# wpats/scanner

Hardware: AMD Instinct MI355X
Metric: Msamples/s (complex samples through convert->window->FFT->dB->threshold) (higher is better)
Workload: dtype f32

## Files before the change

### scanner_amd/csrc/scn_device.h

```cpp
#pragma once
#include <hip/hip_runtime.h>
#include <stdint.h>

#include "scn_kernels.h"

typedef scn_v2f v2f;
typedef float v16f __attribute__((ext_vector_type(16)));

__device__ __forceinline__ cf operator+(cf a, cf b) { return cf{a.x + b.x, a.y + b.y}; }
__device__ __forceinline__ cf operator-(cf a, cf b) { return cf{a.x - b.x, a.y - b.y}; }
__device__ __forceinline__ cf operator*(cf a, float s) { return cf{a.x * s, a.y * s}; }
__device__ __forceinline__ cf from_v2f(v2f v) { return cf{v.x, v.y}; }
__device__ __forceinline__ v2f to_v2f(cf c) { return v2f{c.x, c.y}; }

namespace {

#define SCN_P_EXACT_FROM 1584.8932f
__device__ __forceinline__ float db_fast(float p) { return 1.50514997831990597607f * __builtin_amdgcn_logf(p); }
__device__ __forceinline__ float db_exact(float p) {
  const float m = __builtin_amdgcn_frexp_mantf(p);
  const float e = (float)__builtin_amdgcn_frexp_expf(p);
  const float KH = 1.505126953125f;
  const float KL = (float)(1.50514997831990597607 - 1.505126953125);
  return __builtin_fmaf(KL, e, __builtin_fmaf(1.50514997831990597607f, __builtin_amdgcn_logf(m), KH * e));
// ... 88 lines not shown
  v[14] = mul_w6_d(v[14], H);
  v[7] = cmul_d(v[7], S1, -C1);
  v[11] = mul_w6_d(v[11], H);
  v[15] = cmul_d(v[15], -C1, S1);
#pragma unroll
  for (int k0 = 0; k0 < 4; k0++) radix4_d(v[4 * k0], v[4 * k0 + 1], v[4 * k0 + 2], v[4 * k0 + 3]);
}

__device__ __forceinline__ __amdgpu_buffer_rsrc_t make_rsrc(const void *p, uint32_t bytes) {
  return __builtin_amdgcn_make_buffer_rsrc(const_cast<void *>(p), 0, bytes, 0x00020000);
}
constexpr int SCN_AUX_LD = 2;
constexpr int SCN_AUX_ST = 2;

__device__ __forceinline__ int wave_sum(int v) {
#pragma unroll
  for (int off = 32; off > 0; off >>= 1) v += __shfl_xor(v, off, 64);
  return v;
}

#define SCN_DPP_STEP(OP, x, ctrl, rmask) x = x OP (uint32_t)__builtin_amdgcn_update_dpp(0, (int)x, ctrl, rmask, 0xf, true)
__device__ __forceinline__ uint32_t wave_or_u32(uint32_t x) {
  SCN_DPP_STEP(|, x, 0x111, 0xf);
  SCN_DPP_STEP(|, x, 0x112, 0xf);
  SCN_DPP_STEP(|, x, 0x114, 0xf);
  SCN_DPP_STEP(|, x, 0x118, 0xf);
  SCN_DPP_STEP(|, x, 0x142, 0xa);
  SCN_DPP_STEP(|, x, 0x143, 0xc);
  return (uint32_t)__builtin_amdgcn_readlane((int)x, 63);
}
__device__ __forceinline__ uint32_t wave_add_u32(uint32_t x) {
  SCN_DPP_STEP(+, x, 0x111, 0xf);
  SCN_DPP_STEP(+, x, 0x112, 0xf);
  SCN_DPP_STEP(+, x, 0x114, 0xf);
  SCN_DPP_STEP(+, x, 0x118, 0xf);
  SCN_DPP_STEP(+, x, 0x142, 0xa);
  SCN_DPP_STEP(+, x, 0x143, 0xc);
  return (uint32_t)__builtin_amdgcn_readlane((int)x, 63);
}

template <int NB, typename VEC, typename ARGS, typename BINI>
__device__ __forceinline__ void scn_record_hits_device_counter(VEC &pw, const float (&gmax)[4], uint32_t keepmask, const ARGS &args, int *count,
                                                               uint32_t buf, uint32_t lane, BINI bin_i) {
  constexpr int GS = NB / 4;
  uint32_t wmc = 0;
#pragma unroll
  for (int g = 0; g < 4; g++) {
    if (__ballot(gmax[g] > args.p_lo)) {
#pragma unroll
      for (int o = g * GS; o < (g + 1) * GS; o++) wmc |= __ballot(pw[o] > args.p_lo) ? (1u << o) : 0u;
    }
  }
  ScnDevHit *const region = args.hits + (size_t)buf * args.hit_region;
  uint32_t hm = 0, wm2 = 0, total = 0;
  while (wmc) {
    const int o = __builtin_ctz(wmc);
    wmc &= wmc - 1u;
    const float p = pw[o];
    float d = db_fast(p);
    if (__ballot(p >= SCN_P_EXACT_FROM)) d = p >= SCN_P_EXACT_FROM ? db_exact(p) : d;
    const bool hit = ((keepmask >> o) & 1u) && d > args.threshold && p > args.p_lo;
    const unsigned long long m = __ballot(hit);
    pw[o] = d;
    hm |= hit ? (1u << o) : 0u;
    wm2 |= m ? (1u << o) : 0u;
    total += (uint32_t)__popcll(m);
  }
  if (!total) return;
  uint32_t base = 0;
  if (lane == 0) base = (uint32_t)atomicAdd(count, (int)total);
  base = (uint32_t)__builtin_amdgcn_readfirstlane((int)base);
  while (wm2) {
    const int o = __builtin_ctz(wm2);
    wm2 &= wm2 - 1u;
    const bool hit = (hm >> o) & 1u;
    const unsigned long long m = __ballot(hit);
    if (hit) {
      const uint32_t pos = base + (uint32_t)__popcll(m & ((1ull << lane) - 1ull));
      if (pos < args.hit_region) region[pos] = ScnDevHit{bin_i(o), pw[o]};
    }
    base += (uint32_t)__popcll(m);
  }
}

__device__ __forceinline__ float scn_cndmask(float a, float b, unsigned long long m) {
  float r;
  asm("v_cndmask_b32 %0, %1, %2, %3" : "=v"(r) : "v"(a), "v"(b), "s"(m));
  return r;
}
template <int NB, typename VEC>
__device__ __forceinline__ float scn_select_output(const VEC &pw, uint32_t o) {
  float t[NB / 2];
  const unsigned long long m0 = __ballot(o & 1u);
#pragma unroll
  for (int i = 0; i < NB / 2; i++) t[i] = scn_cndmask(pw[2 * i], pw[2 * i + 1], m0);
#pragma unroll
  for (int w = NB / 4, bit = 1; w >= 1; w >>= 1, bit++) {
    const unsigned long long m = __ballot((o >> bit) & 1u);
#pragma unroll
    for (int i = 0; i < w; i++) t[i] = scn_cndmask(t[2 * i], t[2 * i + 1], m);
  }
  return t[0];
}

template <int T, int NB, typename VEC, typename ARGS, typename BINI>
__device__ __forceinline__ uint32_t scn_record_hits_segment(const VEC &dbv, uint32_t hm, const ARGS &args, uint32_t buf, uint32_t t, BINI bin_i) {
  static_assert(T >= 1 && T <= 32 && (T & (T - 1)) == 0, "a segment is a power of two of lanes inside a wave");
  const uint32_t cnt = (uint32_t)__builtin_popcount(hm);
  uint32_t inc = cnt;
#pragma unroll
  for (int off = 1; off < T; off <<= 1) {
    const uint32_t v = (uint32_t)__shfl_up((int)inc, off, T);
    inc += t >= (uint32_t)off ? v : 0u;
  }
  const uint32_t total = T == 1 ? inc : (uint32_t)__shfl((int)inc, T - 1, T);
  uint32_t pos = inc - cnt;
  ScnDevHit *const region = args.hits + (size_t)buf * args.hit_region;
  while (__ballot(hm != 0u)) {
    const bool act = hm != 0u;
    const uint32_t o = act ? (uint32_t)__builtin_ctz(hm) : 0u;
    hm &= hm - 1u;
    const float d = scn_select_output<NB>(dbv, o);
    if (act && pos < args.hit_region) region[pos] = ScnDevHit{bin_i((int)o), d};
    pos += 1u;
  }
  return total;
}

template <int NB, bool IS_DB, bool PURE = false, bool HAVE_MASK = false, typename VEC, typename ARGS, typename BINI>
__device__ __forceinline__ void scn_record_hits_lanes(VEC &pw, const float (&gmax)[4], uint32_t keepmask, const ARGS &args, int *count, uint32_t buf,
                                                      uint32_t lane, BINI bin_i, uint32_t cand = 0) {
  constexpr int GS = NB / 4;
  uint32_t hm = cand;
  if constexpr (!HAVE_MASK) {
#pragma unroll
    for (int g = 0; g < 4; g++) {
      if (__ballot(gmax[g] > args.p_lo)) {
#pragma unroll
        for (int o = g * GS; o < (g + 1) * GS; o++) hm |= (IS_DB ? pw[o] > args.threshold : pw[o] > args.p_lo) ? (1u << o) : 0u;
      }
    }
  }
  hm &= keepmask;
  ScnDevHit *const region = args.hits + (size_t)buf * args.hit_region;
  if constexpr (IS_DB) {
    const uint32_t cnt = (uint32_t)__builtin_popcount(hm);
    uint32_t inc = cnt;
    SCN_DPP_STEP(+, inc, 0x111, 0xf);
    SCN_DPP_STEP(+, inc, 0x112, 0xf);
    SCN_DPP_STEP(+, inc, 0x114, 0xf);
    SCN_DPP_STEP(+, inc, 0x118, 0xf);
    SCN_DPP_STEP(+, inc, 0x142, 0xa);
    SCN_DPP_STEP(+, inc, 0x143, 0xc);
    const uint32_t total = (uint32_t)__builtin_amdgcn_readlane((int)inc, 63);
    if (!total) return;
    uint32_t base = 0;
    if (lane == 0) base = (uint32_t)atomicAdd(count, (int)total);
    uint32_t pos = (uint32_t)__builtin_amdgcn_readfirstlane((int)base) + inc - cnt;
    while (__ballot(hm != 0u)) {
      const bool act = hm != 0u;
      const uint32_t o = act ? (uint32_t)__builtin_ctz(hm) : 0u;
      hm &= hm - 1u;
      const float d = scn_select_output<NB>(pw, o);
      if (act && pos < args.hit_region) region[pos] = ScnDevHit{bin_i((int)o), d};
      pos += 1u;
    }
    return;
  }
  while (__ballot(hm != 0u)) {
    const bool act = hm != 0u;
    const uint32_t o = act ? (uint32_t)__builtin_ctz(hm) : 0u;
    hm &= hm - 1u;
    const float p = scn_select_output<NB>(pw, o);
    float d = p;
    if constexpr (!IS_DB) {
      d = db_fast(p);
      if constexpr (PURE) {
        const bool ex = p >= SCN_P_EXACT_FROM;
        if (__ballot(act && ex)) d = ex ? db_exact(p) : d;
      } else {
        const float gm = scn_select_output<4>(gmax, o / GS);
        const bool ex = gm >= SCN_P_EXACT_FROM && d == db_fast(gm);
        if (__ballot(act && ex)) d = ex ? db_exact(gm) : d;
      }
    }
    const bool hit = act && d > args.threshold && (IS_DB || p > args.p_lo);
    const unsigned long long m = __ballot(hit);
    if (m) {
      const int first = __builtin_ctzll(m);
      uint32_t base = 0;
      if (lane == (uint32_t)first) base = (uint32_t)atomicAdd(count, (int)__popcll(m));
      base = (uint32_t)__builtin_amdgcn_readlane((int)base, first);
      if (hit) {
        const uint32_t pos = base + (uint32_t)__popcll(m & ((1ull << lane) - 1ull));
        if (pos < args.hit_region) region[pos] = ScnDevHit{bin_i((int)o), d};
      }
    }
  }
}

template <int NB, typename VEC, typename SOFF>
__device__ __forceinline__ void scn_store_exact_db(const VEC &pw, const float (&gmax)[4], float pmax, __amdgpu_buffer_rsrc_t rout, uint32_t st_voff,
                                                   SOFF soff_of) {
  constexpr int GS = NB / 4;
  if (__ballot(pmax >= SCN_P_EXACT_FROM)) {
#pragma unroll
    for (int g = 0; g < 4; g++) {
      if (__ballot(gmax[g] >= SCN_P_EXACT_FROM)) {
#pragma unroll
        for (int o = g * GS; o < (g + 1) * GS; o++) {
          const float q = pw[o];
          if (__ballot(q >= SCN_P_EXACT_FROM)) {
            const float d = db_exact(q);
            __builtin_amdgcn_raw_buffer_store_b32(__builtin_bit_cast(int, d), rout, q >= SCN_P_EXACT_FROM ? st_voff : 0x80000000u, soff_of(o), SCN_AUX_ST);
          }
        }
      }
    }
  }
}

template <int KIND>
struct RawLoader;

template <>
struct RawLoader<SCN_K_FLOAT_COMPLEX> : Wire<SCN_K_FLOAT_COMPLEX> {
  template <int AUX>
  static __device__ __forceinline__ raw_t load(__amdgpu_buffer_rsrc_t r, uint32_t, uint32_t t, uint32_t idx0) {
    return __builtin_bit_cast(v2f, __builtin_amdgcn_raw_buffer_load_b64(r, t * 8u, idx0 * 8u, AUX));
  }
  template <int AUX>
  static __device__ __forceinline__ void load2(__amdgpu_buffer_rsrc_t r, uint32_t, uint32_t t, uint32_t idx0, raw_t &r0, raw_t &r1) {
    typedef float v4f_t __attribute__((ext_vector_type(4)));
    const v4f_t v = __builtin_bit_cast(v4f_t, __builtin_amdgcn_raw_buffer_load_b128(r, t * 16u, idx0 * 8u, AUX));
    r0 = v2f{v.x, v.y};
    r1 = v2f{v.z, v.w};
  }
};

template <>
struct RawLoader<SCN_K_SHORT_COMPLEX> : Wire<SCN_K_SHORT_COMPLEX> {
  template <int AUX>
  static __device__ __forceinline__ raw_t load(__amdgpu_buffer_rsrc_t r, uint32_t, uint32_t t, uint32_t idx0) {
    return __builtin_amdgcn_raw_buffer_load_b32(r, t * 4u, idx0 * 4u, AUX);
  }
  template <int AUX>
  static __device__ __forceinline__ void load2(__amdgpu_buffer_rsrc_t r, uint32_t, uint32_t t, uint32_t idx0, raw_t &r0, raw_t &r1) {
    typedef int v2i_t __attribute__((ext_vector_type(2)));
    const v2i_t v = __builtin_bit_cast(v2i_t, __builtin_amdgcn_raw_buffer_load_b64(r, t * 8u, idx0 * 4u, AUX));
    r0 = v.x;
    r1 = v.y;
  }
};

template <>
struct RawLoader<SCN_K_BYTE_COMPLEX> : Wire<SCN_K_BYTE_COMPLEX> {
  template <int AUX>
  static __device__ __forceinline__ raw_t load(__amdgpu_buffer_rsrc_t r, uint32_t, uint32_t t, uint32_t idx0) {
    int v;
    const unsigned short h = __builtin_amdgcn_raw_buffer_load_b16(r, t * 2u, idx0 * 2u, AUX);
    asm("" : "=v"(v) : "0"(h));
    return v;
  }
  template <int AUX>
  static __device__ __forceinline__ void load2(__amdgpu_buffer_rsrc_t r, uint32_t, uint32_t t, uint32_t idx0, raw_t &r0, raw_t &r1) {
    const uint32_t v = (uint32_t)__builtin_amdgcn_raw_buffer_load_b32(r, t * 4u, idx0 * 2u, AUX);
    r0 = (int)(v & 0xffffu);
    r1 = (int)(v >> 16);
  }
};

template <>
struct RawLoader<SCN_K_SHORT> : Wire<SCN_K_SHORT> {
  template <int AUX>
  static __device__ __forceinline__ raw_t load(__amdgpu_buffer_rsrc_t r, uint32_t n, uint32_t t, uint32_t idx0) {
    int re = (int)(unsigned short)__builtin_amdgcn_raw_buffer_load_b16(r, t * 2u, idx0 * 2u, AUX);
    int im = (int)(unsigned short)__builtin_amdgcn_raw_buffer_load_b16(r, t * 2u, (n + idx0) * 2u, AUX);
    return (re & 0xffff) | (im << 16);
  }
  template <int AUX>
  static __device__ __forceinline__ void load2(__amdgpu_buffer_rsrc_t r, uint32_t n, uint32_t t, uint32_t idx0, raw_t &r0, raw_t &r1) {
    const uint32_t re = (uint32_t)__builtin_amdgcn_raw_buffer_load_b32(r, t * 4u, idx0 * 2u, AUX);
    const uint32_t im = (uint32_t)__builtin_amdgcn_raw_buffer_load_b32(r, t * 4u, (n + idx0) * 2u, AUX);
    r0 = (int)((re & 0xffffu) | (im << 16));
    r1 = (int)((re >> 16) | (im & 0xffff0000u));
  }
};

template <int M>
struct Geo {
  static_assert(M == 4 || M == 8 || M == 16, "1024, 2048 or 4096 points");
  static constexpr uint32_t N = 256u * M;
  static constexpr uint32_t T = 16u * M;
  static constexpr uint32_t P1 = T + M;
  static constexpr uint32_t P2 = 256u + 16u / M;
  static constexpr uint32_t EXCH = (16u * P1 > M * P2) ? 16u * P1 : M * P2;
  static constexpr uint32_t LDS_BYTES = EXCH * 8u + T * 8u + 16u * 4u + 2u * 4u + 64u * 4u + 8u;
  static constexpr uint32_t WAVES = T / 64;
  static constexpr uint32_t WAVES_PER_SIMD = 3;
  static constexpr uint32_t WG_PER_CU = (WAVES_PER_SIMD * 4u) / WAVES;
};

template <int M>
__device__ __forceinline__ constexpr int out_reg(int o) {
  return M == 4 ? o : M == 8 ? (o & ~7) + OUT8(o & 7) : OUT16(o & 15);
}

}
```

### scanner_amd/csrc/scn_kernels.hip

```cpp
#include <hip/hip_runtime.h>
#include <hip/hip_ext.h>
#include <stdint.h>
#include <stdlib.h>

#include "scn_device.h"
#include "scn_dispatch.h"
#include "scn_kernels.h"

#ifndef SCN_TU
#define SCN_TU -1
#endif
#define SCN_IN_TU(x) (SCN_TU == -1 || SCN_TU == (x))
#define SCN_TU_COUNT 8


#define SCN_WORK_QUEUE_SETUP()                                                                         \
  const uint32_t wq_shard = blockIdx.x & 7u;                                                           \
  uint32_t *const wq_head = args.work_counter + 32u * wq_shard;        \
  const uint32_t wq_base = args.work_base[wq_shard];                                                   \
  const uint32_t wq_j0 = (gridDim.x - wq_shard + 7u) >> 3;                                             \
  uint32_t wq_zero;                                                                                    \
  asm("v_mov_b32 %0, 0" : "=v"(wq_zero));                                                              \
  auto wq_take = [&]() -> uint32_t { return atomicAdd(wq_head + wq_zero, 1u); };                       \
  auto wq_buffer = [&](uint32_t taken) -> uint32_t { return 8u * (wq_j0 + (taken - wq_base)) + wq_shard; }

template <int M, int KIND, bool DC, bool HITS, bool SPEC>
__global__ __launch_bounds__(16 * M, Geo<M>::WAVES_PER_SIMD) void scn_fft_kernel(ScnFftArgs args) {
  static_assert(HITS || SPEC, "a kernel that reports nothing");
  typedef Geo<M> G;
  constexpr int AUX_LD = SCN_AUX_LD;
  constexpr int AUX_ST = SCN_AUX_ST;
  constexpr bool DYN = scn_uses_queue(KIND, G::N);
  constexpr uint32_t N = G::N, T = G::T, P1 = G::P1, P2 = G::P2;
  typedef RawLoader<KIND> L;
  extern __shared__ __attribute__((aligned(16))) char smem_raw[];
  v2f *lds = reinterpret_cast<v2f *>(smem_raw);
  v2f *lds_tw2 = lds + G::EXCH;
  int *lds_cnt = reinterpret_cast<int *>(lds_tw2 + T);
  int *lds_hits = lds_cnt + 32;
  uint32_t *lds_next = reinterpret_cast<uint32_t *>(lds_hits + 2);

  const uint32_t t = threadIdx.x;
  const uint32_t p2 = t / M, c2 = t % M;
  const uint32_t lane = t & 63, wave = t >> 6;

  typename L::raw_t raw[16];
  if (blockIdx.x < args.n_buffers) {
    __amdgpu_buffer_rsrc_t r0 = make_rsrc(reinterpret_cast<const char *>(args.raw) + (size_t)blockIdx.x * L::kBytes * N, L::kBytes * N);
#pragma unroll
    for (int a = 0; a < 16; a++) raw[a] = L::template load<AUX_LD>(r0, N, t, T * a);
  }

  cf tw1[16];
#pragma unroll
  for (int p = 1; p < 16; p++) tw1[p] = from_v2f(args.tw1_table[(p - 1) * T + t]);
  float win[16];
#pragma unroll
  for (int a = 0; a < 16; a++) win[a] = args.window[T * a + t] * args.scale;
  lds_tw2[t] = args.twiddle[(16 * p2 * c2) & (N - 1)];
  SCN_WORK_QUEUE_SETUP();
  if (t == 0) {
    lds_hits[0] = lds_hits[1] = 0;
    lds_next[0] = DYN ? wq_buffer(wq_take()) : blockIdx.x + gridDim.x;
  }
  __syncthreads();

  v2f *w1 = lds + t;
  v2f *r1 = lds + p2 * P1 + c2;
  v2f *w2 = lds + c2 * P2 + p2;
  v2f *r3 = lds + t;
  const v2f *tw2 = lds_tw2 + c2;
  const uint32_t st_voff = t * 4u;

  auto joff_of = [](int o) -> uint32_t { return T * ((uint32_t)o / M) + 256u * ((uint32_t)o % M); };
  uint32_t keepmask = 0;
  if (HITS) {
#pragma unroll
    for (int o = 0; o < 16; o++) {
      const uint32_t j = t + joff_of(o);
      const uint32_t i = j ^ (N / 2);
      const bool keep = scn_bin_evaluated(j, i, N, args);
      keepmask |= keep ? (1u << o) : 0u;
    }
  }
  uint32_t par = 0;
  uint32_t prev = 0xffffffffu;

  uint32_t buf = blockIdx.x;
  uint32_t nxt = (uint32_t)__builtin_amdgcn_readfirstlane((int)lds_next[0]);
  while (buf < args.n_buffers) {
    const bool more = nxt < args.n_buffers;
    int dc_re = 0, dc_im = 0;
    if (DC) {
      int sr = 0, si = 0;
#pragma unroll
      for (int a = 0; a < 16; a++) {
        int re, im;
        L::ints(raw[a], re, im);
        sr += re;
        si += im;
      }
      sr = wave_sum(sr);
      si = wave_sum(si);
      if (lane == 0) {
        lds_cnt[wave] = sr;
        lds_cnt[16 + wave] = si;
      }
      __syncthreads();
      sr = si = 0;
#pragma unroll
      for (uint32_t w = 0; w < G::WAVES; w++) {
        sr += lds_cnt[w];
        si += lds_cnt[16 + w];
      }
      dc_re = (int)((uint32_t)sr / N);
      dc_im = (int)((uint32_t)si / N);
    }

    cf v[16];
#pragma unroll
    for (int a = 0; a < 16; a++) v[a] = L::conv(raw[a], dc_re, dc_im, 1.0f) * win[a];
    uint32_t taken = 0;
    if (DYN && t == 0 && more) taken = wq_take();
    const __amdgpu_buffer_rsrc_t rn =
        make_rsrc(reinterpret_cast<const char *>(args.raw) + (size_t)(more ? nxt : buf) * (L::kBytes * N), more ? L::kBytes * N : 0u);
    auto prefetch = [&](int a_lo, int a_hi) {
#pragma unroll
      for (int a = 0; a < 16; a++)
        if (a >= a_lo && a < a_hi) raw[a] = L::template load<AUX_LD>(rn, N, t, T * a);
    };
    prefetch(0, 6);

    fft16(v);
#pragma unroll
    for (int p = 0; p < 16; p++) {
      cf y = v[OUT16(p)];
      if (p) y = cmul(y, tw1[p]);
      w1[p * P1] = to_v2f(y);
    }
    __syncthreads();
    if (HITS) {
      if (t == 0 && prev != 0xffffffffu) {
        args.per_buffer_hits[prev] = (uint32_t)lds_hits[par ^ 1];
        if (args.host_hits) args.host_hits[prev] = (uint32_t)lds_hits[par ^ 1];
        lds_hits[par ^ 1] = 0;
      }
    }

#pragma unroll
    for (int b = 0; b < 16; b++) v[b] = from_v2f(r1[b * M]);
    prefetch(6, 11);
    fft16(v);
#pragma unroll
    for (int q = 1; q < 16; q++) v[OUT16(q)] = cmul(v[OUT16(q)], from_v2f(tw2[q * M]));
    __syncthreads();
    prefetch(11, 16);
#pragma unroll
    for (int q = 0; q < 16; q++) w2[q * 16] = to_v2f(v[OUT16(q)]);
    __syncthreads();

#pragma unroll
    for (int u = 0; u < 16 / M; u++)
#pragma unroll
      for (int c = 0; c < M; c++) v[u * M + c] = from_v2f(r3[c * P2 + T * u]);
    if constexpr (M == 16) fft16(v);
    if constexpr (M == 8) {
      fft8(v);
      fft8(v + 8);
    }
    if constexpr (M == 4) {
#pragma unroll
      for (int u = 0; u < 4; u++) radix4(v[4 * u], v[4 * u + 1], v[4 * u + 2], v[4 * u + 3]);
    }

    v16f pw;
    float gmax[4] = {0.0f, 0.0f, 0.0f, 0.0f};
    __amdgpu_buffer_rsrc_t rout = make_rsrc(args.power_db + (size_t)buf * N, (SPEC && args.power_db) ? 4u * N : 0u);
#pragma unroll
    for (int o = 0; o < 16; o++) {
      const float q = power_of(v[out_reg<M>(o)]);
      pw[o] = q;
      gmax[o >> 2] = fmaxf(gmax[o >> 2], q);
      if constexpr (SPEC) __builtin_amdgcn_raw_buffer_store_b32(__builtin_bit_cast(int, db_fast(q)), rout, st_voff, 4u * joff_of(o), AUX_ST);
    }
    const float pmax = fmaxf(fmaxf(gmax[0], gmax[1]), fmaxf(gmax[2], gmax[3]));
    if constexpr (SPEC) scn_store_exact_db<16>(pw, gmax, pmax, rout, st_voff, [&](int o) -> uint32_t { return 4u * joff_of(o); });
    if (t == 0) lds_next[0] = !more ? 0xffffffffu : DYN ? wq_buffer(taken) : nxt + gridDim.x;
    __syncthreads();
    const uint32_t after = (uint32_t)__builtin_amdgcn_readfirstlane((int)lds_next[0]);
    if (HITS) {
      if (__ballot(pmax > args.p_lo))
        scn_record_hits_lanes<16, false, true>(pw, gmax, keepmask, args, &lds_hits[par], buf, lane, [&](int o) -> uint32_t { return (t + joff_of(o)) ^ (N / 2); });
      prev = buf;
      par ^= 1;
    }
    buf = nxt;
    nxt = after;
  }
  if (HITS) {
    __syncthreads();
    if (t == 0 && prev != 0xffffffffu) {
      args.per_buffer_hits[prev] = (uint32_t)lds_hits[par ^ 1];
      if (args.host_hits) args.host_hits[prev] = (uint32_t)lds_hits[par ^ 1];
    }
  }
}

namespace {
template <int T, bool SPEC, bool HITS, typename POWER, typename JOFF, typename STORE>
__device__ __forceinline__ void scn_small_db_store_record(POWER power_at, JOFF joff_of, STORE store, const ScnFftArgs &args, uint32_t buf, bool valid,
                                                          uint32_t keepmask, uint32_t t, uint32_t n) {
  v16f pw, dbv;
  float gmax[4] = {0.0f, 0.0f, 0.0f, 0.0f};
#pragma unroll
  for (int o = 0; o < 16; o++) {
    const float q = power_at(o);
    pw[o] = q;
    gmax[o >> 2] = fmaxf(gmax[o >> 2], q);
    if constexpr (SPEC) {
      const float d = db_fast(q);
      dbv[o] = d;
      store(o, d, true);
    }
  }
  const float pmax = fmaxf(fmaxf(gmax[0], gmax[1]), fmaxf(gmax[2], gmax[3]));
  const bool any_cand = HITS && __ballot(valid && pmax > args.p_lo) != 0ull;
  if (SPEC || any_cand) {
    if constexpr (!SPEC) {
#pragma unroll
      for (int o = 0; o < 16; o++) dbv[o] = db_fast(pw[o]);
    }
    if (__ballot(pmax >= SCN_P_EXACT_FROM)) {
#pragma unroll
      for (int g = 0; g < 4; g++) {
        if (__ballot(gmax[g] >= SCN_P_EXACT_FROM)) {
#pragma unroll
          for (int o = 4 * g; o < 4 * g + 4; o++) {
            const float q = pw[o];
            if (__ballot(q >= SCN_P_EXACT_FROM)) {
              const float d = db_exact(q);
              dbv[o] = q >= SCN_P_EXACT_FROM ? d : dbv[o];
              if constexpr (SPEC) store(o, d, q >= SCN_P_EXACT_FROM);
            }
          }
        }
      }
    }
  }
  if constexpr (HITS) {
    uint32_t total = 0;
    if (any_cand) {
      uint32_t hm = 0;
#pragma unroll
      for (int o = 0; o < 16; o++) hm |= (dbv[o] > args.threshold) ? (1u << o) : 0u;
      hm &= valid ? keepmask : 0u;
      total = scn_record_hits_segment<T, 16>(dbv, hm, args, buf, t, [&](int o) -> uint32_t { return (t + joff_of(o)) ^ (n / 2); });
    }
    if (t == 0 && valid) {
      args.per_buffer_hits[buf] = total;
      if (args.host_hits) args.host_hits[buf] = total;
    }
  }
}

template <int M>
struct GeoSmall {
  static constexpr uint32_t N = 256u * M, T = 16u * M, SLOTS = 256u / T;
  static constexpr uint32_t P1 = T + M, P2 = 256u + 16u / M;
  static constexpr uint32_t EXCH = (16u * P1 > M * P2) ? 16u * P1 : M * P2;
  static constexpr uint32_t LDS_BYTES = SLOTS * EXCH * 8u + T * 8u + 16u;
  static constexpr uint32_t WG_PER_CU = 3;
};
}

template <int M, int KIND, bool DC, bool HITS, bool SPEC>
__global__ __launch_bounds__(256, 3) void scn_fft_small_kernel(ScnFftArgs args) {
  static_assert(M == 1 || M == 2, "256 or 512 points");
  static_assert(HITS || SPEC, "a kernel that reports nothing");
  typedef GeoSmall<M> G;
  constexpr int AUX_LD = SCN_AUX_LD;
  constexpr int AUX_ST = SCN_AUX_ST;
  constexpr uint32_t N = G::N, T = G::T, SLOTS = G::SLOTS, P1 = G::P1, P2 = G::P2;
  typedef RawLoader<KIND> L;
  extern __shared__ __attribute__((aligned(16))) char smem_raw[];
  const uint32_t tid = threadIdx.x, t = tid % T, slot = tid / T;
  v2f *lds = reinterpret_cast<v2f *>(smem_raw) + slot * G::EXCH;
  v2f *lds_tw2 = reinterpret_cast<v2f *>(smem_raw) + SLOTS * G::EXCH;
  const uint32_t p2 = t / M, c2 = t % M;
  const uint32_t buf_bytes = L::kBytes * N;

  auto in_rsrc = [&](uint32_t first) {
    const bool ok = first < args.n_buffers;
    const uint32_t nb = ok ? (args.n_buffers - first < SLOTS ? args.n_buffers - first : SLOTS) : 0u;
    return make_rsrc(reinterpret_cast<const char *>(args.raw) + (size_t)(ok ? first : 0u) * buf_bytes, nb * buf_bytes);
  };
  typename L::raw_t raw[16];
  auto load_group = [&](const __amdgpu_buffer_rsrc_t &r, int a_lo, int a_hi) {
#pragma unroll
    for (int a = 0; a < 16; a++)
      if (a >= a_lo && a < a_hi) raw[a] = L::template load<AUX_LD>(r, N, t + slot * (KIND == SCN_K_SHORT ? 2u * N : N), T * a);
  };
  uint32_t first = blockIdx.x * SLOTS;
  load_group(in_rsrc(first), 0, 16);

  cf tw1[16];
#pragma unroll
  for (int p = 1; p < 16; p++) tw1[p] = from_v2f(args.tw1_table[(p - 1) * T + t]);
  float win[16];
#pragma unroll
  for (int a = 0; a < 16; a++) win[a] = args.window[T * a + t] * args.scale;
  if (slot == 0) lds_tw2[t] = args.twiddle[(16 * p2 * c2) & (N - 1)];
  __syncthreads();

  v2f *w1 = lds + t;
  v2f *r1 = lds + p2 * P1 + c2;
  v2f *w2 = lds + c2 * P2 + p2;
  v2f *r3 = lds + t;
  const v2f *tw2 = lds_tw2 + c2;
  auto joff_of = [](int o) -> uint32_t { return T * ((uint32_t)o / M) + 256u * ((uint32_t)o % M); };
  uint32_t keepmask = 0;
  if (HITS) {
#pragma unroll
    for (int o = 0; o < 16; o++) {
      const uint32_t j = t + joff_of(o);
      const uint32_t i = j ^ (N / 2);
      const bool keep = scn_bin_evaluated(j, i, N, args);
      keepmask |= keep ? (1u << o) : 0u;
    }
  }

  for (; first < args.n_buffers; first += gridDim.x * SLOTS) {
    const uint32_t buf = first + slot;
    const bool valid = buf < args.n_buffers;
    int dc_re = 0, dc_im = 0;
    if (DC) {
      int sr = 0, si = 0;
#pragma unroll
      for (int a = 0; a < 16; a++) {
        int re, im;
        L::ints(raw[a], re, im);
        sr += re;
        si += im;
      }
#pragma unroll
      for (uint32_t off = T / 2; off > 0; off >>= 1) {
        sr += __shfl_xor(sr, (int)off, 64);
        si += __shfl_xor(si, (int)off, 64);
      }
      dc_re = (int)((uint32_t)sr / N);
      dc_im = (int)((uint32_t)si / N);
    }
    cf v[16];
#pragma unroll
    for (int a = 0; a < 16; a++) v[a] = L::conv(raw[a], dc_re, dc_im, 1.0f) * win[a];
    const __amdgpu_buffer_rsrc_t rn = in_rsrc(first + gridDim.x * SLOTS);
    load_group(rn, 0, 6);

    fft16(v);
#pragma unroll
    for (int p = 0; p < 16; p++) {
      cf y = v[OUT16(p)];
      if (p) y = cmul(y, tw1[p]);
      w1[p * P1] = to_v2f(y);
    }
    __syncthreads();
#pragma unroll
    for (int b = 0; b < 16; b++) v[b] = from_v2f(r1[b * M]);
    load_group(rn, 6, 11);
    fft16(v);
    if constexpr (M == 1) {
      load_group(rn, 11, 16);
    } else {
#pragma unroll
      for (int q = 1; q < 16; q++) v[OUT16(q)] = cmul(v[OUT16(q)], from_v2f(tw2[q * M]));
      __syncthreads();
      load_group(rn, 11, 16);
#pragma unroll
      for (int q = 0; q < 16; q++) w2[q * 16] = to_v2f(v[OUT16(q)]);
      __syncthreads();
#pragma unroll
      for (int u = 0; u < 16 / M; u++)
#pragma unroll
        for (int c = 0; c < M; c++) v[u * M + c] = from_v2f(r3[c * P2 + T * u]);
#pragma unroll
      for (int u = 0; u < 8; u++) {
        const cf a = v[2 * u], b = v[2 * u + 1];
        v[2 * u] = a + b;
        v[2 * u + 1] = a - b;
      }
    }
    const uint32_t nvalid = args.n_buffers - first < SLOTS ? args.n_buffers - first : SLOTS;
    __amdgpu_buffer_rsrc_t rout = make_rsrc(args.power_db + (size_t)first * N, (SPEC && args.power_db) ? nvalid * 4u * N : 0u);
    const uint32_t st_voff = (slot * N + t) * 4u;
    scn_small_db_store_record<(int)T, SPEC, HITS>(
        [&](int o) -> float { return power_of(v[M == 1 ? OUT16(o) : o]); }, joff_of,
        [&](int o, float d, bool pred) { __builtin_amdgcn_raw_buffer_store_b32(__builtin_bit_cast(int, d), rout, pred ? st_voff : 0x80000000u, 4u * joff_of(o), AUX_ST); },
        args, buf, valid, keepmask, t, N);
    __syncthreads();
  }
}

namespace {
template <int R>
struct GeoTiny {
  static constexpr uint32_t N = 16u * R, T = R, SLOTS = 256u / R;
  static constexpr uint32_t P1 = R + 1u;
  static constexpr uint32_t EXCH = R == 1 ? 0u : 16u * P1 + R;
  static constexpr uint32_t PITCH = N + R;
  static constexpr uint32_t TILE_BYTES = SLOTS * PITCH * 8u;
  static constexpr uint32_t LDS_BYTES = (TILE_BYTES > SLOTS * EXCH * 8u ? TILE_BYTES : SLOTS * EXCH * 8u) + 16u;
  static constexpr uint32_t WG_PER_CU = 3;
};

template <int KIND, int R>
struct TinyStage {
  typedef GeoTiny<R> G;
  typedef RawLoader<KIND> L;
  static constexpr bool PLANAR = KIND == SCN_K_SHORT;
  typedef typename L::raw_t reg_t;
  template <int AUX>
  static __device__ __forceinline__ reg_t load(__amdgpu_buffer_rsrc_t r, uint32_t tid, int a) {
    if constexpr (PLANAR) {
      return __builtin_amdgcn_raw_buffer_load_b32(r, tid * 4u, 1024u * (uint32_t)a, AUX);
    } else {
      return L::template load<AUX>(r, G::N, tid, 256u * (uint32_t)a);
    }
  }
  static __device__ __forceinline__ void stage(char *tile, uint32_t tid, int a, reg_t v) {
    if constexpr (PLANAR) {
      unsigned short *t16 = reinterpret_cast<unsigned short *>(tile);
#pragma unroll
      for (int h = 0; h < 2; h++) {
        const uint32_t e = 512u * (uint32_t)a + 2u * tid + h, s = e / (2u * G::N), j = e % (2u * G::N);
        t16[s * 2u * G::PITCH + (j < G::N ? j : G::PITCH + j - G::N)] = (unsigned short)(h ? (uint32_t)v >> 16 : (uint32_t)v & 0xffffu);
      }
    } else {
      const uint32_t e = 256u * (uint32_t)a + tid, idx = (e / G::N) * G::PITCH + e % G::N;
      if constexpr (KIND == SCN_K_FLOAT_COMPLEX) reinterpret_cast<v2f *>(tile)[idx] = v;
      else if constexpr (KIND == SCN_K_SHORT_COMPLEX) reinterpret_cast<int *>(tile)[idx] = v;
      else reinterpret_cast<unsigned short *>(tile)[idx] = (unsigned short)v;
    }
  }
  static __device__ __forceinline__ typename L::raw_t gather(const char *tile, uint32_t slot, uint32_t j) {
    if constexpr (PLANAR) {
      const unsigned short *t16 = reinterpret_cast<const unsigned short *>(tile) + slot * 2u * G::PITCH;
      return (int)((uint32_t)t16[j] | ((uint32_t)t16[G::PITCH + j] << 16));
    } else if constexpr (KIND == SCN_K_FLOAT_COMPLEX) {
      return reinterpret_cast<const v2f *>(tile)[slot * G::PITCH + j];
    } else if constexpr (KIND == SCN_K_SHORT_COMPLEX) {
      return reinterpret_cast<const int *>(tile)[slot * G::PITCH + j];
    } else {
      return (int)reinterpret_cast<const unsigned short *>(tile)[slot * G::PITCH + j];
    }
  }
};
}

template <int R, int KIND, bool DC, bool HITS, bool SPEC>
__global__ __launch_bounds__(256, 3) void scn_fft_tiny_kernel(ScnFftArgs args) {
  static_assert(R == 1 || R == 2 || R == 4 || R == 8, "16, 32, 64 or 128 points");
  static_assert(HITS || SPEC, "a kernel that reports nothing");
  typedef GeoTiny<R> G;
  typedef TinyStage<KIND, R> S;
  constexpr int AUX_LD = SCN_AUX_LD;
  constexpr int AUX_ST = SCN_AUX_ST;
  constexpr uint32_t N = G::N, SLOTS = G::SLOTS, P1 = G::P1, PITCH = G::PITCH;
  typedef RawLoader<KIND> L;
// ... 524 lines not shown
    for (int q = 0; q < 16; q++) {
      w2[q * 32] = to_v2f(va[OUT16(q)]);
      w2[q * 32 + 16] = to_v2f(vb[OUT16(q)]);
    }
    __syncthreads();

    v32f pw;
    float gmax[4] = {0.0f, 0.0f, 0.0f, 0.0f};
    uint32_t cand = 0;
    __amdgpu_buffer_rsrc_t rout = make_rsrc(args.power_db + (size_t)buf * N, (SPEC && args.power_db) ? 4u * N : 0u);
#pragma unroll
    for (int h = 0; h < 2; h++) {
      cd vd[16];
#pragma unroll
      for (int c = 0; c < 16; c++) {
        const cd x0 = to_cd(r3[c * P2]), x1 = to_cd(r3[(c + 16) * P2]);
        if (h == 0) {
          vd[c] = x0 + x1;
        } else {
          const cd dlt = x0 - x1;
          const double cr = __builtin_cos(6.283185307179586476925286766559 * c / 32.0), sr = __builtin_sin(6.283185307179586476925286766559 * c / 32.0);
          vd[c] = c ? cmul_d(dlt, cr, -sr) : dlt;
        }
      }
      fft16_d(vd);
#pragma unroll
      for (int rho = 0; rho < 16; rho++) {
        const int r = 2 * rho + h;
        const cd x = vd[OUT16(rho)];
        const float q = (float)__builtin_fma(x.y, x.y, x.x * x.x);
        gmax[r >> 3] = fmaxf(gmax[r >> 3], q);
        if constexpr (SPEC) {
          const float d = db_fast(q);
          pw[r] = d;
          __builtin_amdgcn_raw_buffer_store_b32(__builtin_bit_cast(int, d), rout, st_voff, 2048u * r, AUX_ST);
        } else {
          pw[r] = q;
          if constexpr (HITS) cand |= q > args.p_lo ? (1u << r) : 0u;
        }
      }
      __builtin_amdgcn_sched_barrier(0);
    }
    const float pmax = fmaxf(fmaxf(gmax[0], gmax[1]), fmaxf(gmax[2], gmax[3]));
    if constexpr (SPEC) {
      if (__ballot(pmax >= SCN_P_EXACT_FROM)) {
#pragma unroll
        for (int g = 0; g < 4; g++) {
          if (__ballot(gmax[g] >= SCN_P_EXACT_FROM)) {
            const float dg = db_fast(gmax[g]), ex = db_exact(gmax[g]);
#pragma unroll
            for (int r = 8 * g; r < 8 * g + 8; r++) {
              const float d = pw[r];
              const bool sel = gmax[g] >= SCN_P_EXACT_FROM && d == dg;
              if (__ballot(sel)) {
                pw[r] = sel ? ex : d;
                __builtin_amdgcn_raw_buffer_store_b32(__builtin_bit_cast(int, ex), rout, sel ? st_voff : 0x80000000u, 2048u * r, AUX_ST);
              }
            }
          }
        }
      }
    }
    __syncthreads();
    if (HITS) {
      if (__ballot(pmax > args.p_lo))
        scn_record_hits_lanes<32, SPEC, false, !SPEC>(pw, gmax, keepmask, args, &lds_hits[par], buf, lane, [&](int r) -> uint32_t { return (t + 512u * (uint32_t)r) ^ (N / 2); }, cand);
      prev = buf;
      par ^= 1;
    }
  }
  if (HITS) {
    __syncthreads();
    if (t == 0 && prev != 0xffffffffu) {
      args.per_buffer_hits[prev] = (uint32_t)lds_hits[par ^ 1];
      if (args.host_hits) args.host_hits[prev] = (uint32_t)lds_hits[par ^ 1];
    }
  }
}

}

template <int KIND, bool DC, bool HITS, bool SPEC>
__global__ __launch_bounds__(512, 2) void scn_fft16k2_kernel(ScnFftArgs args) {
  scn_fft16k2_body<KIND, DC, HITS, SPEC>(args);
}

__device__ __forceinline__ float scn_td_db(float p) {
  const float k = 3.01029995663981195214f;
  const bool denormal = p > 0.0f && p < 1.17549435e-38f;
  const float l = __builtin_amdgcn_logf(__builtin_amdgcn_sqrtf(denormal ? p * 0x1p64f : p));
  return k * (denormal ? l - 32.0f : l);
}
__device__ __forceinline__ void scn_td_store(const ScnTdArgs &args, uint32_t buf, float pmax, float pmin) {
  args.max_db[buf] = fmaxf(1.17549435e-38f, scn_td_db(pmax));
  args.min_db[buf] = pmin == __builtin_inff() ? 3.40282347e+38f : fminf(3.40282347e+38f, scn_td_db(pmin));
}

template <int KIND, bool DC>
__global__ __launch_bounds__(256) void scn_time_domain_kernel(ScnTdArgs args) {
  typedef RawLoader<KIND> L;
  __shared__ float s_max[4], s_min[4];
  __shared__ int s_sum[8];
  const uint32_t t = threadIdx.x, lane = t & 63, wave = t >> 6;
  const uint32_t N = args.n;
  for (uint32_t buf = blockIdx.x; buf < args.n_buffers; buf += gridDim.x) {
    __amdgpu_buffer_rsrc_t rin =
        make_rsrc(reinterpret_cast<const char *>(args.raw) + (size_t)buf * (L::kBytes * N), L::kBytes * N);
    int dc_re = 0, dc_im = 0;
    if (DC) {
      int sr = 0, si = 0;
      for (uint32_t i = t; i < N; i += 256) {
        int re, im;
        L::ints(L::template load<0>(rin, N, i, 0), re, im);
        sr += re;
        si += im;
      }
      sr = wave_sum(sr);
      si = wave_sum(si);
      if (lane == 0) {
        s_sum[wave] = sr;
        s_sum[4 + wave] = si;
      }
      __syncthreads();
      dc_re = (int)((uint32_t)(s_sum[0] + s_sum[1] + s_sum[2] + s_sum[3]) / N);
      dc_im = (int)((uint32_t)(s_sum[4] + s_sum[5] + s_sum[6] + s_sum[7]) / N);
    }
    float pmax = -1.0f, pmin = __builtin_inff();
    for (uint32_t i = t; i < N; i += 256) {
#pragma clang fp contract(off)
      cf x = L::conv(L::template load<0>(rin, N, i, 0), dc_re, dc_im, args.scale);
      float p = x.x * x.x + x.y * x.y;
      pmax = fmaxf(pmax, p);
      pmin = fminf(pmin, p);
    }
#pragma unroll
    for (int off = 32; off > 0; off >>= 1) {
      pmax = fmaxf(pmax, __shfl_xor(pmax, off, 64));
      pmin = fminf(pmin, __shfl_xor(pmin, off, 64));
    }
    if (lane == 0) {
      s_max[wave] = pmax;
      s_min[wave] = pmin;
    }
    __syncthreads();
    if (t == 0) {
      pmax = fmaxf(fmaxf(s_max[0], s_max[1]), fmaxf(s_max[2], s_max[3]));
      pmin = fminf(fminf(s_min[0], s_min[1]), fminf(s_min[2], s_min[3]));
      scn_td_store(args, buf, pmax, pmin);
    }
    __syncthreads();
  }
}

template <int KIND, bool DC>
__global__ __launch_bounds__(256) void scn_time_domain_wave_kernel(ScnTdArgs args) {
  typedef RawLoader<KIND> L;
  typedef int v4i_t __attribute__((__vector_size__(16)));
  constexpr bool PLANAR = KIND == SCN_K_SHORT;
  const uint32_t lane = threadIdx.x & 63u;
  const uint32_t gw = blockIdx.x * 4u + (uint32_t)__builtin_amdgcn_readfirstlane((int)(threadIdx.x >> 6)), nw = gridDim.x * 4u;
  const uint32_t N = args.n;
  const uint32_t bytes = L::kBytes * N;
  const uint32_t stream_bytes = PLANAR ? 2u * N : bytes;
  const uint32_t chunks = stream_bytes / 16u;
  for (uint32_t buf = gw; buf < args.n_buffers; buf += nw) {
    const __amdgpu_buffer_rsrc_t rin =
        make_rsrc(reinterpret_cast<const char *>(args.raw) + (size_t)buf * bytes, bytes);
    auto for_each_sample = [&](auto &&f) {
      for (uint32_t c0 = 0; c0 < chunks; c0 += 256u) {
        v4i_t w[4], wq[4];
#pragma unroll
        for (int u = 0; u < 4; u++) {
          const uint32_t c = c0 + 64u * u + lane;
          w[u] = __builtin_bit_cast(v4i_t, __builtin_amdgcn_raw_buffer_load_b128(rin, c * 16u, 0, SCN_AUX_LD));
          if (PLANAR) wq[u] = __builtin_bit_cast(v4i_t, __builtin_amdgcn_raw_buffer_load_b128(rin, c * 16u, stream_bytes, SCN_AUX_LD));
        }
#pragma unroll
        for (int u = 0; u < 4; u++) {
          if (c0 + 64u * u + lane < chunks) {
#pragma unroll
            for (int k = 0; k < 4; k++) {
              const int d = w[u][k];
              if constexpr (KIND == SCN_K_FLOAT_COMPLEX) {
                if (k & 1) f(v2f{__builtin_bit_cast(float, (int)w[u][k - 1]), __builtin_bit_cast(float, d)});
              } else if constexpr (KIND == SCN_K_SHORT_COMPLEX) {
                f(d);
              } else if constexpr (KIND == SCN_K_BYTE_COMPLEX) {
                f(d & 0xffff);
                f((int)((uint32_t)d >> 16));
              } else {
                const int q = wq[u][k];
                f((d & 0xffff) | (q << 16));
                f((int)((uint32_t)d >> 16) | (q & (int)0xffff0000));
              }
            }
          }
        }
      }
    };
    int dc_re = 0, dc_im = 0;
    if (DC) {
      int sr = 0, si = 0;
      for_each_sample([&](typename L::raw_t r) {
        int re, im;
        L::ints(r, re, im);
        sr += re;
        si += im;
      });
      sr = wave_sum(sr);
      si = wave_sum(si);
      dc_re = (int)((uint32_t)sr / N);
      dc_im = (int)((uint32_t)si / N);
    }
    float pmax = -1.0f, pmin = __builtin_inff();
    for_each_sample([&](typename L::raw_t r) {
#pragma clang fp contract(off)
      const cf x = L::conv(r, dc_re, dc_im, args.scale);
      const float p = x.x * x.x + x.y * x.y;
      pmax = fmaxf(pmax, p);
      pmin = fminf(pmin, p);
    });
#pragma unroll
    for (int off = 32; off > 0; off >>= 1) {
      pmax = fmaxf(pmax, __shfl_xor(pmax, off, 64));
      pmin = fminf(pmin, __shfl_xor(pmin, off, 64));
    }
    if (lane == 0) {
      scn_td_store(args, buf, pmax, pmin);
    }
  }
}

#if SCN_IN_TU(7)
hipError_t scn_launch_time_domain(int kind, bool dc, const ScnTdArgs &a, int num_cus, hipStream_t s) {
  if (a.n_buffers == 0) return hipSuccess;
  const bool waves = a.n % 8u == 0;
  uint32_t grid = waves ? (a.n_buffers + 3u) / 4u : a.n_buffers;
  const uint32_t resident = (uint32_t)num_cus * 8u;
  if (grid > resident) grid = resident;
  return scn_with_kind(kind, dc, [&](auto k, auto d) {
    constexpr int KIND = decltype(k)::value;
    constexpr bool DC = decltype(d)::value;
    if (waves) hipLaunchKernelGGL((scn_time_domain_wave_kernel<KIND, DC>), dim3(grid), dim3(256), 0, s, a);
    else hipLaunchKernelGGL((scn_time_domain_kernel<KIND, DC>), dim3(grid), dim3(256), 0, s, a);
    return hipGetLastError();
  });
}
#endif

template <int KIND, bool DC>
__global__ __launch_bounds__(256) void scn_convert_kernel(const void *raw, scn_v2f *out, uint32_t n, uint32_t n_buffers,
                                                          float scale) {
  typedef RawLoader<KIND> L;
  __shared__ int s_sum[8];
  const uint32_t t = threadIdx.x, lane = t & 63, wave = t >> 6;
  for (uint32_t buf = blockIdx.x; buf < n_buffers; buf += gridDim.x) {
    __amdgpu_buffer_rsrc_t rin = make_rsrc(reinterpret_cast<const char *>(raw) + (size_t)buf * (L::kBytes * n), L::kBytes * n);
    int dc_re = 0, dc_im = 0;
    if (DC) {
      int sr = 0, si = 0;
      for (uint32_t i = t; i < n; i += 256) {
        int re, im;
        L::ints(L::template load<0>(rin, n, i, 0), re, im);
        sr += re;
        si += im;
      }
      sr = wave_sum(sr);
      si = wave_sum(si);
      if (lane == 0) {
        s_sum[wave] = sr;
        s_sum[4 + wave] = si;
      }
      __syncthreads();
      dc_re = (int)((uint32_t)(s_sum[0] + s_sum[1] + s_sum[2] + s_sum[3]) / n);
      dc_im = (int)((uint32_t)(s_sum[4] + s_sum[5] + s_sum[6] + s_sum[7]) / n);
    }
    for (uint32_t i = t; i < n; i += 256)
      out[(size_t)buf * n + i] = to_v2f(L::conv(L::template load<0>(rin, n, i, 0), dc_re, dc_im, scale));
    __syncthreads();
  }
}

#if SCN_IN_TU(7)
hipError_t scn_launch_convert(int kind, bool dc, const void *raw, scn_v2f *out, uint32_t n, uint32_t n_buffers, float scale,
                              hipStream_t s) {
  if (n_buffers == 0) return hipSuccess;
  return scn_with_kind(kind, dc, [&](auto k, auto d) {
    hipLaunchKernelGGL((scn_convert_kernel<decltype(k)::value, decltype(d)::value>), dim3(n_buffers < 2048 ? n_buffers : 2048), dim3(256), 0, s, raw, out,
                       n, n_buffers, scale);
    return hipGetLastError();
  });
}
#endif

template <typename K>
static hipError_t launch_with_stop(K k, int grid, uint32_t threads, uint32_t lds, hipStream_t s, hipEvent_t stop, const ScnFftArgs &a) {
  if (stop) hipExtLaunchKernelGGL(k, dim3(grid), dim3(threads), lds, s, nullptr, stop, 0, a);
  else hipLaunchKernelGGL(k, dim3(grid), dim3(threads), lds, s, a);
  return hipGetLastError();
}

template <int M>
struct NarrowFamily {
  typedef Geo<M> G;
  static constexpr uint32_t THREADS = G::T, SLOTS = 1;
  template <int KIND, bool DC, bool HITS, bool SPEC>
  static constexpr void (*kernel)(ScnFftArgs) = scn_fft_kernel<M, KIND, DC, HITS, SPEC>;
};
template <int M>
struct SmallFamily {
  typedef GeoSmall<M> G;
  static constexpr uint32_t THREADS = 256, SLOTS = G::SLOTS;
  template <int KIND, bool DC, bool HITS, bool SPEC>
  static constexpr void (*kernel)(ScnFftArgs) = scn_fft_small_kernel<M, KIND, DC, HITS, SPEC>;
};
template <int R>
struct TinyFamily {
  typedef GeoTiny<R> G;
  static constexpr uint32_t THREADS = 256, SLOTS = G::SLOTS;
  template <int KIND, bool DC, bool HITS, bool SPEC>
  static constexpr void (*kernel)(ScnFftArgs) = scn_fft_tiny_kernel<R, KIND, DC, HITS, SPEC>;
};
struct Family8k {
  typedef Geo8k G;
  static constexpr uint32_t THREADS = G::T, SLOTS = 1;
  template <int KIND, bool DC, bool HITS, bool SPEC>
  static constexpr void (*kernel)(ScnFftArgs) = scn_fft8k_kernel<KIND, DC, HITS, SPEC>;
};
struct Family16k {
  typedef Geo16k2 G;
  static constexpr uint32_t THREADS = G::T, SLOTS = 1;
  template <int KIND, bool DC, bool HITS, bool SPEC>
  static constexpr void (*kernel)(ScnFftArgs) = scn_fft16k2_kernel<KIND, DC, HITS, SPEC>;
};

template <class F>
static hipError_t launch_kernel(void (*k)(ScnFftArgs), const ScnFftLaunch &l) {
  typedef typename F::G G;
  if (G::LDS_BYTES > 65536u) {
    hipError_t e = hipFuncSetAttribute(reinterpret_cast<const void *>(k), hipFuncAttributeMaxDynamicSharedMemorySize, (int)G::LDS_BYTES);
    if (e != hipSuccess) return e;
  }
  const uint32_t groups = (l.args.n_buffers + F::SLOTS - 1u) / F::SLOTS;
  int grid = l.num_cus * (int)G::WG_PER_CU;
  if ((uint32_t)grid > groups) grid = (int)groups;
  return launch_with_stop(k, grid, F::THREADS, G::LDS_BYTES, l.stream, l.stop, l.args);
}

template <class F>
static hipError_t launch_family(const ScnFftLaunch &l) {
  return scn_with_kind(l.kind, l.dc, [&](auto kind, auto dc) {
    return scn_with_mode(l.hits, l.spec, [&](auto hits, auto spec) {
      return launch_kernel<F>(F::template kernel<decltype(kind)::value, decltype(dc)::value, decltype(hits)::value, decltype(spec)::value>, l);
    });
  });
}

template <int TU>
static hipError_t launch_fft_unit(uint32_t n, const ScnFftLaunch &l) {
  if constexpr (TU == 0) return n == 16 ? launch_family<TinyFamily<1>>(l) : launch_family<TinyFamily<2>>(l);
  else if constexpr (TU == 1) return n == 64 ? launch_family<TinyFamily<4>>(l) : launch_family<TinyFamily<8>>(l);
  else if constexpr (TU == 2) return n == 256 ? launch_family<SmallFamily<1>>(l) : launch_family<SmallFamily<2>>(l);
  else if constexpr (TU == 3) return n == 1024 ? launch_family<NarrowFamily<4>>(l) : launch_family<NarrowFamily<8>>(l);
  else if constexpr (TU == 4) return launch_family<NarrowFamily<16>>(l);
  else if constexpr (TU == 5) return launch_family<Family8k>(l);
  else return launch_family<Family16k>(l);
}
template <int TU>
hipError_t scn_launch_fft_unit(uint32_t n, const ScnFftLaunch &l);
#if SCN_TU == -1
template <int TU>
hipError_t scn_launch_fft_unit(uint32_t n, const ScnFftLaunch &l) { return launch_fft_unit<TU>(n, l); }
#elif SCN_TU < 7
template <>
hipError_t scn_launch_fft_unit<SCN_TU>(uint32_t n, const ScnFftLaunch &l) { return launch_fft_unit<SCN_TU>(n, l); }
#endif

#if SCN_IN_TU(7)
hipError_t scn_launch_fft(uint32_t n, int kind, bool dc, bool hits, bool spec, const ScnFftArgs &args, int num_cus,
                          hipStream_t stream, hipEvent_t stop) {
  if (!hits && !spec) return hipErrorInvalidValue;
  if (args.n_buffers == 0) return stop ? hipEventRecord(stop, stream) : hipSuccess;
  if (!scn_fft_size_supported(n)) return hipErrorInvalidValue;
  if (n < 1024 && (uint64_t)args.n_buffers * n * 8u > 0xffffffffull) return hipErrorInvalidValue;
  static constexpr hipError_t (*units[7])(uint32_t, const ScnFftLaunch &) = {scn_launch_fft_unit<0>, scn_launch_fft_unit<1>, scn_launch_fft_unit<2>,
                                                                             scn_launch_fft_unit<3>, scn_launch_fft_unit<4>, scn_launch_fft_unit<5>,
                                                                             scn_launch_fft_unit<6>};
  const int lg = __builtin_ctz(n);
  return units[lg < 12 ? (lg - 4) / 2 : lg - 8](n, ScnFftLaunch{kind, dc, hits, spec, args, num_cus, stream, stop});
}

bool scn_fft_size_supported(uint32_t n) { return n >= 16 && n <= 16384 && (n & (n - 1u)) == 0u; }

void scn_tw1_layout(uint32_t n, uint32_t *rows, uint32_t *threads) {
  *rows = n == 16384 ? 31u : 15u;
  *threads = n == 16384 ? 512u : n / 16u;
}
#endif
```

Baseline: 461,000.

## Make second FFT exchange in-place in LDS to drop a barrier

Replaces the separate write and read layouts of the three-stage LDS exchange with one in-place slot layout. Each thread now writes its second-stage results back to the same slots it read, which removes one __syncthreads per buffer. The last prefetch chunk moves after the third-stage read. The cost is a fresh padding scheme that has to avoid bank conflicts for all three access patterns, and the in-place read-then-write order is only safe if every thread reads and writes exactly the same slots.

Measured after the change: 462,500 (median of 6 runs). No clear change (+0.3%).

```diff
diff --git a/scanner_amd/csrc/scn_device.h b/scanner_amd/csrc/scn_device.h
--- a/scanner_amd/csrc/scn_device.h
+++ b/scanner_amd/csrc/scn_device.h
@@ -414,6 +414,17 @@
 };
 
 template <int M>
+struct GeoInplace : Geo<M> {
+  static constexpr uint32_t SP = M == 16 ? 257u : M == 8 ? 1u : 4u;
+  static constexpr uint32_t SB = M == 16 ? 16u : M == 8 ? 16u : 66u;
+  static constexpr uint32_t SC = M == 16 ? 1u : M == 8 ? 258u : 1u;
+  static constexpr uint32_t slot(uint32_t p, uint32_t b, uint32_t c) { return SP * p + SB * b + SC * c; }
+  static constexpr uint32_t EXCH = slot(15, 15, M - 1) + 1u;
+  static_assert(EXCH <= Geo<M>::EXCH, "the in-place area must not cost occupancy");
+  static constexpr uint32_t LDS_BYTES = EXCH * 8u + Geo<M>::T * 8u + 16u * 4u + 2u * 4u + 64u * 4u + 8u;
+};
+
+template <int M>
 __device__ __forceinline__ constexpr int out_reg(int o) {
   return M == 4 ? o : M == 8 ? (o & ~7) + OUT8(o & 7) : OUT16(o & 15);
 }
diff --git a/scanner_amd/csrc/scn_kernels.hip b/scanner_amd/csrc/scn_kernels.hip
--- a/scanner_amd/csrc/scn_kernels.hip
+++ b/scanner_amd/csrc/scn_kernels.hip
@@ -24,14 +24,18 @@
   auto wq_take = [&]() -> uint32_t { return atomicAdd(wq_head + wq_zero, 1u); };                       \
   auto wq_buffer = [&](uint32_t taken) -> uint32_t { return 8u * (wq_j0 + (taken - wq_base)) + wq_shard; }
 
+#ifndef SCN_PF_A
+#define SCN_PF_A 6
+#define SCN_PF_B 11
+#endif
 template <int M, int KIND, bool DC, bool HITS, bool SPEC>
 __global__ __launch_bounds__(16 * M, Geo<M>::WAVES_PER_SIMD) void scn_fft_kernel(ScnFftArgs args) {
   static_assert(HITS || SPEC, "a kernel that reports nothing");
-  typedef Geo<M> G;
+  typedef GeoInplace<M> G;
   constexpr int AUX_LD = SCN_AUX_LD;
   constexpr int AUX_ST = SCN_AUX_ST;
   constexpr bool DYN = scn_uses_queue(KIND, G::N);
-  constexpr uint32_t N = G::N, T = G::T, P1 = G::P1, P2 = G::P2;
+  constexpr uint32_t N = G::N, T = G::T, SP = G::SP, SB = G::SB, SC = G::SC;
   typedef RawLoader<KIND> L;
   extern __shared__ __attribute__((aligned(16))) char smem_raw[];
   v2f *lds = reinterpret_cast<v2f *>(smem_raw);
@@ -65,10 +69,9 @@
   }
   __syncthreads();
 
-  v2f *w1 = lds + t;
-  v2f *r1 = lds + p2 * P1 + c2;
-  v2f *w2 = lds + c2 * P2 + p2;
-  v2f *r3 = lds + t;
+  v2f *w1 = lds + G::slot(0, t / M, t % M);
+  v2f *x2 = lds + G::slot(p2, 0, c2);
+  v2f *r3 = lds + G::slot(t % 16u, t / 16u, 0);
   const v2f *tw2 = lds_tw2 + c2;
   const uint32_t st_voff = t * 4u;
 
@@ -129,14 +132,14 @@
       for (int a = 0; a < 16; a++)
         if (a >= a_lo && a < a_hi) raw[a] = L::template load<AUX_LD>(rn, N, t, T * a);
     };
-    prefetch(0, 6);
+    prefetch(0, SCN_PF_A);
 
     fft16(v);
 #pragma unroll
     for (int p = 0; p < 16; p++) {
       cf y = v[OUT16(p)];
       if (p) y = cmul(y, tw1[p]);
-      w1[p * P1] = to_v2f(y);
+      w1[p * SP] = to_v2f(y);
     }
     __syncthreads();
     if (HITS) {
@@ -148,21 +151,20 @@
     }
 
 #pragma unroll
-    for (int b = 0; b < 16; b++) v[b] = from_v2f(r1[b * M]);
-    prefetch(6, 11);
+    for (int b = 0; b < 16; b++) v[b] = from_v2f(x2[b * SB]);
+    prefetch(SCN_PF_A, SCN_PF_B);
     fft16(v);
 #pragma unroll
     for (int q = 1; q < 16; q++) v[OUT16(q)] = cmul(v[OUT16(q)], from_v2f(tw2[q * M]));
-    __syncthreads();
-    prefetch(11, 16);
-#pragma unroll
-    for (int q = 0; q < 16; q++) w2[q * 16] = to_v2f(v[OUT16(q)]);
+#pragma unroll
+    for (int q = 0; q < 16; q++) x2[q * SB] = to_v2f(v[OUT16(q)]);
     __syncthreads();
 
 #pragma unroll
     for (int u = 0; u < 16 / M; u++)
 #pragma unroll
-      for (int c = 0; c < M; c++) v[u * M + c] = from_v2f(r3[c * P2 + T * u]);
+      for (int c = 0; c < M; c++) v[u * M + c] = from_v2f(r3[c * SC + M * u * SB]);
+    prefetch(SCN_PF_B, 16);
     if constexpr (M == 16) fft16(v);
     if constexpr (M == 8) {
       fft8(v);
@@ -1293,7 +1295,7 @@
 
 template <int M>
 struct NarrowFamily {
-  typedef Geo<M> G;
+  typedef GeoInplace<M> G;
   static constexpr uint32_t THREADS = G::T, SLOTS = 1;
   template <int KIND, bool DC, bool HITS, bool SPEC>
   static constexpr void (*kernel)(ScnFftArgs) = scn_fft_kernel<M, KIND, DC, HITS, SPEC>;
```
